# thangktran/HardwareAwareOptimalQuantumCircuitCuttingAndKnitting

Hardware: AMD Instinct MI355X
Metric: subcircuit-instances/s (full-knit wall time = ms_per_step), syc 32 p=2 (higher is better)
Workload: dtype f64

## Files before the change

hardwareawareoptimalquantumcircuitcuttingandknitting_amd/csrc/qknit_prep.hip:

```cpp
#include <hip/hip_runtime.h>

#include <cstdint>
#include <string>

#include "internal.h"

namespace {

typedef double d4_t __attribute__((ext_vector_type(4)));
typedef double d2_t __attribute__((ext_vector_type(2)));

constexpr int PK = 64;
constexpr int PCT = 128;
constexpr int PNP = 16;
constexpr int PTH = 512;
constexpr int XLD = PCT + 2;
constexpr int PG_BLK = 10;
constexpr int PPG = PG_BLK * 256;
constexpr int PPA = PPG;
constexpr int PPB = PPG + PK * PNP;
__host__ __device__ constexpr int prep_tri(int bi, int bj) { return bi * 4 - bi * (bi - 1) / 2 + (bj - bi); }

struct PrepSide {
    const double* Wt;
    const double* q;
    int64_t ldq;
    int64_t N;
    int R;
    double* X;
    const double* P;
};

struct PrepArgs {
    PrepSide s[2];
    int K;
    int split;
    double* part;
};

#ifndef QK_PREP_RS
#define QK_PREP_RS 16
#endif
constexpr int PRS = QK_PREP_RS;
constexpr int PRPW = PRS / 8;
static_assert(PRS % 8 == 0 && PRS >= 8, "stage rows: a multiple of 8 (8 waves)");
#ifndef QK_PREP_NS
#define QK_PREP_NS 2
#endif
#ifndef QK_PREP_WG_PER_CU
#define QK_PREP_WG_PER_CU 2
#endif
#ifndef QK_COMPRESS_COLS
#define QK_COMPRESS_COLS 1
#endif
#ifndef QK_PREP_EXP
#define QK_PREP_EXP 0
#endif
constexpr int PNS = QK_PREP_NS;
#ifndef QK_PREP_QPAD
#define QK_PREP_QPAD 16
#endif
#ifndef QK_PREP_WPAD
#define QK_PREP_WPAD 16
#endif
constexpr int QLD = PCT + QK_PREP_QPAD;
constexpr int WLD = PK + QK_PREP_WPAD;
struct PrepStage {
    double q[PRS][QLD];
    double w[PRS][WLD];
};
union PrepLds {
    PrepStage st[PNS];
    double x[PK][XLD];
};

__device__ __forceinline__ void prep_glds(const double* src, double* lds_row) {
    __builtin_amdgcn_global_load_lds(reinterpret_cast<const void*>(src),
                                     reinterpret_cast<__attribute__((address_space(3))) void*>(
                                         reinterpret_cast<uintptr_t>(lds_row)),
                                     16, 0, 0);
}

__device__ __forceinline__ void prep_vmwait(int n) {
    switch (n < 15 ? n : 15) {
#define QK_PW(k) case k: asm volatile("s_waitcnt vmcnt(" #k ")" ::: "memory"); break;
        QK_PW(0) QK_PW(1) QK_PW(2) QK_PW(3) QK_PW(4) QK_PW(5) QK_PW(6) QK_PW(7)
        QK_PW(8) QK_PW(9) QK_PW(10) QK_PW(11) QK_PW(12) QK_PW(13) QK_PW(14) QK_PW(15)
#undef QK_PW
    }
}

__global__ __launch_bounds__(PTH, 2 * QK_PREP_WG_PER_CU) void qk_prep_operands_kernel(PrepArgs a) {
    __shared__ __attribute__((aligned(16))) PrepLds L;
    const int tid = threadIdx.x, lane = tid & 63, wave = tid >> 6;
    const int l16 = lane & 15, l4 = lane >> 4;
    const int K = a.K;
    int gi0, gj0, gi1 = -1, gj1 = -1;
    switch (wave) {
        case 4: gi0 = 0, gj0 = 1, gi1 = 0, gj1 = 2; break;
        case 5: gi0 = 0, gj0 = 3, gi1 = 1, gj1 = 2; break;
        case 6: gi0 = 1, gj0 = 3; break;
        case 7: gi0 = 2, gj0 = 3; break;
        default: gi0 = gj0 = wave; break;
    }
    gi0 = __builtin_amdgcn_readfirstlane(gi0), gj0 = __builtin_amdgcn_readfirstlane(gj0);
    gi1 = __builtin_amdgcn_readfirstlane(gi1), gj1 = __builtin_amdgcn_readfirstlane(gj1);
    const int wave_s = __builtin_amdgcn_readfirstlane(wave);
    for (int sd = 0; sd < 2; ++sd) {
        const PrepSide& S = a.s[sd];
        const int R = S.R;
        const int nst = (R + PRS - 1) / PRS;
        const int64_t tiles = S.N / PCT;
        d4_t g0 = {0, 0, 0, 0}, g1 = {0, 0, 0, 0}, u = {0, 0, 0, 0};
        const bool mine = !a.split || (int)(blockIdx.x & 1) == sd;
        const int64_t t_first = a.split ? (int64_t)(blockIdx.x >> 1) : (int64_t)blockIdx.x;
        const int64_t t_step = a.split ? (int64_t)(gridDim.x >> 1) : (int64_t)gridDim.x;
        for (int64_t t = mine ? t_first : tiles; t < tiles; t += t_step) {
            const int64_t c0 = t * PCT;
            int nload[PNS];
            auto issue = [&](int st) {
                PrepStage& P = L.st[st % PNS];
                int n = 0;
#pragma unroll
                for (int h = 0; h < PRPW; ++h) {
                    const int rl = PRPW * wave_s + h, r = st * PRS + rl;
                    if (r < R) {
                        prep_glds(S.q + (int64_t)r * S.ldq + c0 + 2 * lane, &P.q[rl][0]);
                        ++n;
                        if (2 * lane < K) prep_glds(S.Wt + (int64_t)r * K + 2 * lane, &P.w[rl][0]);
                        ++n;
                    }
                }
                nload[st % PNS] = n;
            };
            asm volatile("s_waitcnt lgkmcnt(0)" ::: "memory");
            __builtin_amdgcn_s_barrier();
            for (int st = 0; st < PNS - 1 && st < nst; ++st) issue(st);
            d4_t x[4];
#pragma unroll
            for (int i = 0; i < 4; ++i) x[i] = (d4_t){0, 0, 0, 0};
            for (int st = 0; st < ((QK_PREP_EXP & 4) ? 0 : nst); ++st) {
                int after = 0;
                for (int d = st + 1; d < st + PNS - 1 && d < nst; ++d) after += nload[d % PNS];
                prep_vmwait(after);
                asm volatile("s_waitcnt lgkmcnt(0)" ::: "memory");
                __builtin_amdgcn_s_barrier();
                const PrepStage& P = L.st[st % PNS];
                double qb[PRS / 4], wa[PRS / 4][4];
#pragma unroll
                for (int kk = 0; kk < PRS / 4; ++kk) {
                    const int rl = 4 * kk + l4;
                    const bool rv = st * PRS + rl < R;
                    qb[kk] = rv ? P.q[rl][16 * wave + l16] : 0.0;
#pragma unroll
                    for (int i = 0; i < 4; ++i) {
                        const int k = 16 * i + l16;
                        wa[kk][i] = (rv && k < K) ? P.w[rl][k] : 0.0;
                    }
                }
                if (st + PNS - 1 < nst) issue(st + PNS - 1);
#pragma unroll
                for (int kk = 0; kk < PRS / 4; ++kk)
#pragma unroll
                    for (int i = 0; i < 4; ++i) x[i] = __builtin_amdgcn_mfma_f64_16x16x4f64(wa[kk][i], qb[kk], x[i], 0, 0, 0);
            }
            const bool probes = S.P != nullptr && wave < 4;
            constexpr int PPB = 8;
            const double* pp = probes ? S.P + (int64_t)l16 * S.N + c0 + l4 : nullptr;
            double pxn[PPB];
#pragma unroll
            for (int j = 0; j < PPB; ++j) pxn[j] = probes ? pp[4 * j] : 0.0;
            asm volatile("s_waitcnt lgkmcnt(0)" ::: "memory");
            __builtin_amdgcn_s_barrier();
#pragma unroll
            for (int i = 0; i < 4; ++i)
#pragma unroll
                for (int rr = 0; rr < 4; ++rr) L.x[16 * i + l4 + 4 * rr][16 * wave + l16] = x[i][rr];
            asm volatile("s_waitcnt lgkmcnt(0)" ::: "memory");
            __builtin_amdgcn_s_barrier();
            for (int s8 = 0; s8 < ((QK_PREP_EXP & 1) ? 0 : PCT / 4); s8 += PPB) {
                double px[PPB];
#pragma unroll
                for (int j = 0; j < PPB; ++j) px[j] = pxn[j];
                if (probes && s8 + PPB < PCT / 4) {
#pragma unroll
                    for (int j = 0; j < PPB; ++j) pxn[j] = pp[4 * (s8 + PPB + j)];
                }
                if (wave < 4) {
#pragma unroll
                    for (int j = 0; j < PPB; ++j) {
                        const double av = L.x[16 * gi0 + l16][4 * (s8 + j) + l4];
                        g0 = __builtin_amdgcn_mfma_f64_16x16x4f64(av, av, g0, 0, 0, 0);
                        if (probes) u = __builtin_amdgcn_mfma_f64_16x16x4f64(av, px[j], u, 0, 0, 0);
                    }
                } else {
#pragma unroll
                    for (int j = 0; j < PPB; ++j) {
                        const int c = 4 * (s8 + j) + l4;
                        const double a0 = L.x[16 * gi0 + l16][c];
                        const double b0 = L.x[16 * gj0 + l16][c];
                        g0 = __builtin_amdgcn_mfma_f64_16x16x4f64(a0, b0, g0, 0, 0, 0);
                        if (gi1 >= 0) {
                            const double a1 = gi1 == gi0 ? a0 : L.x[16 * gi1 + l16][c];
                            const double b1 = L.x[16 * gj1 + l16][c];
                            g1 = __builtin_amdgcn_mfma_f64_16x16x4f64(a1, b1, g1, 0, 0, 0);
                        }
                    }
                }
            }
            if (!(QK_PREP_EXP & 2)) {
                d2_t z[8];
#pragma unroll
                for (int v = 0; v < 8; ++v) z[v] = *reinterpret_cast<const d2_t*>(&L.x[8 * wave_s + v][2 * lane]);
#pragma unroll
                for (int v = 0; v < 8; ++v)
                    if (8 * wave_s + v < K) *reinterpret_cast<d2_t*>(S.X + (int64_t)(8 * wave_s + v) * S.N + c0 + 2 * lane) = z[v];
            }
        }
        double* p = sd == 0 ? a.part + (int64_t)blockIdx.x * PPA
                            : a.part + (int64_t)gridDim.x * PPA + (int64_t)blockIdx.x * PPB;
#pragma unroll
        for (int rr = 0; rr < 4; ++rr) {
            const int e = (l4 + 4 * rr) * 16 + l16;
            p[prep_tri(gi0, gj0) * 256 + e] = g0[rr];
            if (gi1 >= 0) p[prep_tri(gi1, gj1) * 256 + e] = g1[rr];
            if (sd == 1 && wave < 4) p[PPG + (16 * wave + l4 + 4 * rr) * PNP + l16] = u[rr];
        }
    }
}

constexpr int PRW = 16;
__global__ __launch_bounds__(64 * PRW) void qk_prep_reduce_kernel(const double* __restrict__ part, int nblk,
                                                                  int K, double* __restrict__ GA,
                                                                  double* __restrict__ GB, double* __restrict__ U) {
    __shared__ double acc[PRW][64];
    const int lane = threadIdx.x & 63, grp = threadIdx.x >> 6;
    const int e = blockIdx.x * 64 + lane;
    int sd = -1, off = 0;
    double* dst = nullptr;
    double* mirror = nullptr;
    if (e < 2 * PPG) {
        sd = e < PPG ? 0 : 1;
        off = e - sd * PPG;
        const int blk = off >> 8;
        const int bi = blk < 4 ? 0 : blk < 7 ? 1 : blk < 9 ? 2 : 3;
        const int bj = bi + blk - prep_tri(bi, bi);
        const int r = 16 * bi + ((off >> 4) & 15), c = 16 * bj + (off & 15);
        if (r < K && c < K) {
            double* G = sd == 0 ? GA : GB;
            dst = G + r * K + c;
            if (bi != bj) mirror = G + c * K + r;
        }
    } else if (e < 2 * PPG + PNP * K) {
        const int f = e - 2 * PPG;
        sd = 1, off = PPG + f, dst = U + f;
    }
    if (!dst) sd = -1;
    double s = 0.0;
    if (sd >= 0) {
        const int PPART = sd == 0 ? PPA : PPB;
        const double* p = part + (sd == 0 ? 0 : (int64_t)nblk * PPA) + off;
        double t[8] = {0, 0, 0, 0, 0, 0, 0, 0};
        int b = grp;
        for (; b + 31 * PRW < nblk; b += 32 * PRW) {
            double v[32];
#pragma unroll
            for (int u = 0; u < 32; ++u) v[u] = p[(int64_t)(b + PRW * u) * PPART];
#pragma unroll
            for (int u = 0; u < 32; ++u) t[u & 7] += v[u];
        }
        for (; b < nblk; b += PRW) t[0] += p[(int64_t)b * PPART];
        s = ((t[0] + t[1]) + (t[2] + t[3])) + ((t[4] + t[5]) + (t[6] + t[7]));
    }
    acc[grp][lane] = s;
    __syncthreads();
    if (grp == 0 && dst) {
        double v[PRW];
#pragma unroll
        for (int w = 0; w < PRW; ++w) v[w] = acc[w][lane];
#pragma unroll
        for (int h = PRW / 2; h >= 1; h >>= 1)
#pragma unroll
            for (int w = 0; w < h; ++w) v[w] += v[w + h];
        *dst = v[0];
        if (mirror) *mirror = v[0];
    }
}

__global__ __launch_bounds__(256) void qk_compress_kernel(int K, int rmax, const double* __restrict__ TA,
                                                          const double* __restrict__ XA, int64_t NA, int64_t ldxa,
                                                          double* __restrict__ A2, int64_t lda2,
                                                          const double* __restrict__ TB,
                                                          const double* __restrict__ XB, int64_t NB, int64_t ldxb,
                                                          double* __restrict__ B2, int64_t ldb2) {
    __shared__ double T[8][PK];
    __shared__ double part[4][8][64];
    const bool bs = blockIdx.y == 1;
    const double* Tg = bs ? TB : TA;
    const double* X = bs ? XB : XA;
    double* out = bs ? B2 : A2;
    const int64_t N = bs ? NB : NA, ld = bs ? ldxb : ldxa, ldo = bs ? ldb2 : lda2;
    const int l = threadIdx.x & 63;
    const int q = __builtin_amdgcn_readfirstlane(threadIdx.x >> 6);
    auto load = [&](int64_t c0, double (&xv)[16]) {
        const int64_t c = c0 + l;
#pragma unroll
        for (int u = 0; u < 16; ++u) {
            const int k = 16 * q + u;
            const double* row = X + (int64_t)k * ld;
            xv[u] = (k < K && c < N) ? row[c] : 0.0;
        }
    };
    double xv[16];
    int64_t c0 = (int64_t)blockIdx.x * 64;
    if (c0 < N) load(c0, xv);
    {
        const int n = rmax * K, e0 = threadIdx.x, e1 = threadIdx.x + 256;
        const double t0 = e0 < n ? Tg[e0] : 0.0, t1 = e1 < n ? Tg[e1] : 0.0;
        if (e0 < n) T[e0 / K][e0 % K] = t0;
        if (e1 < n) T[e1 / K][e1 % K] = t1;
    }
    __syncthreads();
    for (; c0 < N; c0 += (int64_t)gridDim.x * 64) {
        double acc[8] = {0, 0, 0, 0, 0, 0, 0, 0};
#pragma unroll
        for (int u = 0; u < 16; ++u)
#pragma unroll
            for (int j = 0; j < 8; ++j)
                if (j < rmax && 16 * q + u < K) acc[j] = fma(T[j][16 * q + u], xv[u], acc[j]);
#pragma unroll
        for (int j = 0; j < 8; ++j) part[q][j][l] = acc[j];
        __syncthreads();
        for (int e = threadIdx.x; e < 8 * 64; e += 256) {
            const int j = e >> 6, cc = e & 63;
            if (j < rmax && c0 + cc < N)
                out[(int64_t)j * ldo + c0 + cc] = (part[0][j][cc] + part[1][j][cc]) + (part[2][j][cc] + part[3][j][cc]);
        }
        __syncthreads();
        if (c0 + (int64_t)gridDim.x * 64 < N) load(c0 + (int64_t)gridDim.x * 64, xv);
    }
}

constexpr int PCW = 16;
__global__ __launch_bounds__(64) void qk_compress_cols_kernel(int K, int rmax, const double* __restrict__ TA,
                                                              const double* __restrict__ XA, int64_t NA, int64_t ldxa,
                                                              double* __restrict__ A2, int64_t lda2,
                                                              const double* __restrict__ TB,
                                                              const double* __restrict__ XB, int64_t NB, int64_t ldxb,
                                                              double* __restrict__ B2, int64_t ldb2) {
    const bool bs = blockIdx.y == 1;
    const double* Tg = bs ? TB : TA;
    const double* X = bs ? XB : XA;
    double* out = bs ? B2 : A2;
    const int64_t N = bs ? NB : NA, ld = bs ? ldxb : ldxa, ldo = bs ? ldb2 : lda2;
    const int64_t c = ((int64_t)blockIdx.x * 64 + threadIdx.x) * 2;
    if ((int64_t)blockIdx.x * 128 >= N) return;
    const int64_t cl = c < N ? c : N - 2;
    d2_t acc[8];
#pragma unroll
    for (int j = 0; j < 8; ++j) acc[j] = (d2_t){0.0, 0.0};
    __shared__ __attribute__((aligned(16))) double Tt[PK][8];
    d2_t buf[2][PCW];
    auto load = [&](int ch, d2_t (&b)[PCW]) {
#pragma unroll
        for (int u = 0; u < PCW; ++u) {
            const int k = min(ch * PCW + u, K - 1);
            b[u] = *reinterpret_cast<const d2_t*>(X + (int64_t)k * ld + cl);
        }
    };
    const int nch = (K + PCW - 1) / PCW;
    {
        double tv[PK * 8 / 64];
#pragma unroll
        for (int i = 0; i < PK * 8 / 64; ++i) {
            const int e = threadIdx.x + 64 * i, k = e >> 3, j = e & 7;
            tv[i] = Tg[min(j, rmax - 1) * K + min(k, K - 1)];
        }
        load(0, buf[0]);
#pragma unroll
        for (int i = 0; i < PK * 8 / 64; ++i) {
            const int e = threadIdx.x + 64 * i, k = e >> 3, j = e & 7;
            Tt[k][j] = (k < K && j < rmax) ? tv[i] : 0.0;
        }
    }
    __syncthreads();
    if (c >= N) return;
#pragma unroll
    for (int ch = 0; ch < PK / PCW; ++ch) {
        if (ch >= nch) break;
        if (ch + 1 < nch) load(ch + 1, buf[(ch + 1) & 1]);
#pragma unroll
        for (int u = 0; u < PCW; ++u) {
            const int k = ch * PCW + u;
            double t[8];
#pragma unroll
            for (int h = 0; h < 4; ++h) {
                const d2_t tv = *reinterpret_cast<const d2_t*>(&Tt[k][2 * h]);
                t[2 * h] = tv.x;
                t[2 * h + 1] = tv.y;
            }
#pragma unroll
            for (int j = 0; j < 8; ++j) {
                acc[j].x = fma(t[j], buf[ch & 1][u].x, acc[j].x);
                acc[j].y = fma(t[j], buf[ch & 1][u].y, acc[j].y);
            }
        }
    }
#pragma unroll
    for (int j = 0; j < 8; ++j)
        if (j < rmax) *reinterpret_cast<d2_t*>(out + (int64_t)j * ldo + c) = acc[j];
}

constexpr int PV_GRID = 128;
constexpr int PV_PART = 8 * 16;

constexpr int CV_COLS = 512;
__global__ __launch_bounds__(256) void qk_compress_v_kernel(int K, int rmax, const double* __restrict__ TA,
                                                            const double* __restrict__ XA, int64_t NA, int64_t ldxa,
                                                            double* __restrict__ A2, int64_t lda2,
                                                            const double* __restrict__ TB,
                                                            const double* __restrict__ XB, int64_t NB, int64_t ldxb,
                                                            double* __restrict__ B2, int64_t ldb2,
                                                            const double* __restrict__ P, int64_t ldp,
                                                            double* __restrict__ vpart, int nA_wg) {
    const int tid = threadIdx.x, lane = tid & 63, wave = tid >> 6;
    const bool bs = (int)blockIdx.x >= nA_wg;
    const int64_t wg = bs ? (int64_t)blockIdx.x - nA_wg : (int64_t)blockIdx.x;
    const double* Tg = bs ? TB : TA;
    const double* X = bs ? XB : XA;
    double* out = bs ? B2 : A2;
    const int64_t N = bs ? NB : NA, ld = bs ? ldxb : ldxa, ldo = bs ? ldb2 : lda2;
    const int64_t base = wg * CV_COLS + wave * 128;
    const int64_t c = base + 2 * lane;
    const bool valid = c < N;
    const int64_t cl = valid ? c : N - 2;
    __shared__ __attribute__((aligned(16))) double Tt[PK][8];
    __shared__ __attribute__((aligned(16))) double Bt[4][8][128 + 2];
    __shared__ double Vw[4][PV_PART];
    d2_t acc[8];
#pragma unroll
    for (int j = 0; j < 8; ++j) acc[j] = (d2_t){0.0, 0.0};
    d2_t buf[2][PCW];
    auto load = [&](int ch, d2_t (&b)[PCW]) {
#pragma unroll
        for (int u = 0; u < PCW; ++u) {
            const int k = min(ch * PCW + u, K - 1);
            b[u] = *reinterpret_cast<const d2_t*>(X + (int64_t)k * ld + cl);
        }
    };
    const int nch = (K + PCW - 1) / PCW;
    {
        double tv[2];
#pragma unroll
        for (int i = 0; i < 2; ++i) {
            const int e = tid + 256 * i, k = e >> 3, j = e & 7;
            tv[i] = Tg[min(j, rmax - 1) * K + min(k, K - 1)];
        }
        if (base < N) load(0, buf[0]);
#pragma unroll
        for (int i = 0; i < 2; ++i) {
            const int e = tid + 256 * i, k = e >> 3, j = e & 7;
            Tt[k][j] = (k < K && j < rmax) ? tv[i] : 0.0;
        }
    }
    __syncthreads();
    if (base < N) {
#pragma unroll
        for (int ch = 0; ch < PK / PCW; ++ch) {
            if (ch >= nch) break;
            if (ch + 1 < nch) load(ch + 1, buf[(ch + 1) & 1]);
#pragma unroll
            for (int u = 0; u < PCW; ++u) {
                const int k = ch * PCW + u;
                double t[8];
#pragma unroll
                for (int h = 0; h < 4; ++h) {
                    const d2_t tv = *reinterpret_cast<const d2_t*>(&Tt[k][2 * h]);
                    t[2 * h] = tv.x;
                    t[2 * h + 1] = tv.y;
                }
#pragma unroll
                for (int j = 0; j < 8; ++j) {
                    acc[j].x = fma(t[j], buf[ch & 1][u].x, acc[j].x);
                    acc[j].y = fma(t[j], buf[ch & 1][u].y, acc[j].y);
                }
            }
        }
        if (valid) {
#pragma unroll
            for (int j = 0; j < 8; ++j)
                if (j < rmax) *reinterpret_cast<d2_t*>(out + (int64_t)j * ldo + c) = acc[j];
        }
    }
    if (!bs) return;
#pragma unroll
    for (int j = 0; j < 8; ++j) {
        const d2_t v = (valid && j < rmax) ? acc[j] : (d2_t){0.0, 0.0};
        *reinterpret_cast<d2_t*>(&Bt[wave][j][2 * lane]) = v;
    }
    __syncthreads();
    const int i16 = lane & 15, k4 = lane >> 4;
    d4_t va = {0.0, 0.0, 0.0, 0.0};
    if (base < N) {
        constexpr int VB = 8;
        const double* pr = P + (int64_t)i16 * ldp;
#pragma unroll
        for (int s0 = 0; s0 < 32; s0 += VB) {
            double pb[VB];
#pragma unroll
            for (int s = 0; s < VB; ++s) {
                const int64_t col = base + 4 * (s0 + s) + k4;
                pb[s] = col < N ? pr[col] : 0.0;
            }
#pragma unroll
            for (int s = 0; s < VB; ++s) {
                const double a = i16 < 8 ? Bt[wave][i16][4 * (s0 + s) + k4] : 0.0;
                va = __builtin_amdgcn_mfma_f64_16x16x4f64(a, pb[s], va, 0, 0, 0);
            }
        }
    }
#pragma unroll
    for (int r = 0; r < 2; ++r) Vw[wave][(k4 + 4 * r) * 16 + i16] = va[r];
    __syncthreads();
    if (tid < PV_PART)
        vpart[wg * PV_PART + tid] = (Vw[0][tid] + Vw[1][tid]) + (Vw[2][tid] + Vw[3][tid]);
}

__global__ __launch_bounds__(256) void qk_probe_v_kernel(int rmax, const double* __restrict__ B2, int64_t ldb2,
                                                         int64_t NB, const double* __restrict__ P, int64_t ldp,
                                                         double* __restrict__ vpart) {
    const int tid = threadIdx.x, lane = tid & 63, wave = tid >> 6;
    double acc[8][4];
#pragma unroll
    for (int jj = 0; jj < 8; ++jj)
#pragma unroll
        for (int q = 0; q < 4; ++q) acc[jj][q] = 0.0;
    struct Col {
        double b[8], pv[4];
    };
    const int64_t step = (int64_t)gridDim.x * 64;
    auto fetch = [&](int64_t c, Col& x) {
        const int64_t cc = c < NB ? c : NB - 1;
#pragma unroll
        for (int jj = 0; jj < 8; ++jj) x.b[jj] = B2[(int64_t)min(jj, rmax - 1) * ldb2 + cc];
#pragma unroll
        for (int q = 0; q < 4; ++q) x.pv[q] = P[(int64_t)(4 * wave + q) * ldp + cc];
    };
    auto mac = [&](const Col& x) {
#pragma unroll
        for (int jj = 0; jj < 8; ++jj)
#pragma unroll
            for (int q = 0; q < 4; ++q) acc[jj][q] = fma(x.b[jj], x.pv[q], acc[jj][q]);
    };
    int64_t c = (int64_t)blockIdx.x * 64 + lane;
    if (c < NB) {
        Col x0, x1;
        fetch(c, x0);
        for (;; c += 2 * step) {
            fetch(c + step, x1);
            __builtin_amdgcn_sched_barrier(0);
            mac(x0);
            if (c + step >= NB) break;
            fetch(c + 2 * step, x0);
            __builtin_amdgcn_sched_barrier(0);
            mac(x1);
            if (c + 2 * step >= NB) break;
        }
    }
#pragma unroll
    for (int jj = 0; jj < 8; ++jj)
#pragma unroll
        for (int q = 0; q < 4; ++q) {
            double v = acc[jj][q];
#pragma unroll
            for (int s = 1; s < 64; s <<= 1) v += __shfl_xor(v, s, 64);
            acc[jj][q] = jj < rmax ? v : 0.0;
        }
    double* out = vpart + (int64_t)blockIdx.x * PV_PART;
    if (lane < 32) {
        const int j8 = lane >> 2, q = lane & 3;
        double v = 0.0;
#pragma unroll
        for (int jj = 0; jj < 8; ++jj)
#pragma unroll
            for (int qq = 0; qq < 4; ++qq)
                if (jj == j8 && qq == q) v = acc[jj][qq];
        out[j8 * 16 + 4 * wave + q] = v;
    }
}

__global__ __launch_bounds__(256) void qk_probe_d_kernel(int K, int rmax, const double* __restrict__ XA, int64_t ldx,
                                                         int64_t NA, const double* __restrict__ A2, int64_t lda2,
                                                         const double* __restrict__ U,
                                                         const double* __restrict__ vpart, int gv,
                                                         double* __restrict__ epart) {
    __shared__ double Us[PK][PNP];
    __shared__ double Vs[16][PNP];
    __shared__ double ep[4][2 * PNP];
    const int tid = threadIdx.x, lane = tid & 63, wave = tid >> 6, l16 = lane & 15, l4 = lane >> 4;
    {
        __shared__ double vh[PV_PART];
        const int e = tid & (PV_PART - 1), h = tid >> 7;
        double t[16];
#pragma unroll
        for (int u = 0; u < 16; ++u) t[u] = 0.0;
        int b = h;
        for (; b + 30 < gv; b += 32) {
            double v[16];
#pragma unroll
            for (int u = 0; u < 16; ++u) v[u] = vpart[(int64_t)(b + 2 * u) * PV_PART + e];
#pragma unroll
            for (int u = 0; u < 16; ++u) t[u] += v[u];
        }
        for (; b < gv; b += 2) t[0] += vpart[(int64_t)b * PV_PART + e];
#pragma unroll
        for (int w = 8; w >= 1; w >>= 1)
#pragma unroll
            for (int u = 0; u < w; ++u) t[u] += t[u + w];
        if (h == 1) vh[e] = t[0];
        __syncthreads();
        if (h == 0) Vs[e / 16][e % 16] = -(t[0] + vh[e]);
        else Vs[8 + e / 16][e % 16] = 0.0;
    }
    for (int e = tid; e < PK * PNP; e += 256) Us[e / PNP][e % PNP] = (e / PNP) < K ? U[e] : 0.0;
    __syncthreads();
    double e2 = 0.0, f2 = 0.0;
    for (int64_t cb = (int64_t)blockIdx.x * 4 + wave; cb * 16 < NA; cb += (int64_t)gridDim.x * 4) {
        const int64_t c = cb * 16 + l16;
        double av[PK / 4], a2[2];
#pragma unroll
        for (int kk = 0; kk < PK / 4; ++kk) av[kk] = XA[(int64_t)min(4 * kk + l4, K - 1) * ldx + c];
#pragma unroll
        for (int jj = 0; jj < 2; ++jj) a2[jj] = A2[(int64_t)min(4 * jj + l4, rmax - 1) * lda2 + c];
        d4_t acc = {0, 0, 0, 0};
#pragma unroll
        for (int kk = 0; kk < PK / 4; ++kk)
            acc = __builtin_amdgcn_mfma_f64_16x16x4f64(av[kk], Us[4 * kk + l4][l16], acc, 0, 0, 0);
#pragma unroll
        for (int rr = 0; rr < 4; ++rr) f2 = fma(acc[rr], acc[rr], f2);
#pragma unroll
        for (int jj = 0; jj < 2; ++jj)
            acc = __builtin_amdgcn_mfma_f64_16x16x4f64(a2[jj], Vs[4 * jj + l4][l16], acc, 0, 0, 0);
#pragma unroll
        for (int rr = 0; rr < 4; ++rr) e2 = fma(acc[rr], acc[rr], e2);
    }
    e2 += __shfl_xor(e2, 16, 64);
    e2 += __shfl_xor(e2, 32, 64);
    f2 += __shfl_xor(f2, 16, 64);
    f2 += __shfl_xor(f2, 32, 64);
    if (l4 == 0) {
        ep[wave][l16] = e2;
        ep[wave][PNP + l16] = f2;
    }
    __syncthreads();
    if (tid < 2 * PNP)
        epart[(int64_t)blockIdx.x * 2 * PNP + tid] = ep[0][tid] + ep[1][tid] + ep[2][tid] + ep[3][tid];
}

constexpr int PE = 2 * PNP;

__global__ __launch_bounds__(256) void qk_probe_accept_kernel(const double* __restrict__ epart, int n,
                                                              const int32_t* __restrict__ r_dev, double tol,
                                                              double rel_tol, double* __restrict__ e2_out,
                                                              int32_t* __restrict__ k_out, double* __restrict__ err_out,
                                                              int64_t* __restrict__ tally = nullptr) {
    __shared__ double acc[256];
    const int tid = threadIdx.x, p = tid % PE;
    constexpr int STEP = 256 / PE;
    double s8[8] = {0, 0, 0, 0, 0, 0, 0, 0};
    int b = tid / PE;
    for (; b + 31 * STEP < n; b += 32 * STEP) {
        double v[32];
#pragma unroll
        for (int u = 0; u < 32; ++u) v[u] = epart[(int64_t)(b + u * STEP) * PE + p];
#pragma unroll
        for (int u = 0; u < 32; ++u) s8[u & 7] += v[u];
    }
    for (; b < n; b += STEP) s8[0] += epart[(int64_t)b * PE + p];
    const double s = ((s8[0] + s8[1]) + (s8[2] + s8[3])) + ((s8[4] + s8[5]) + (s8[6] + s8[7]));
    acc[tid] = s;
    __syncthreads();
    for (int w = 128; w >= PE; w >>= 1) {
        if (tid < w) acc[tid] += acc[tid + w];
        __syncthreads();
    }
    if (tid < PE && e2_out) e2_out[tid] = acc[tid];
    if (tid == 0 && k_out) {
        double m = 0.0, f = 0.0;
        for (int q = 0; q < PNP; ++q) {
            m = fmax(m, acc[q]);
            f = fmax(f, acc[PNP + q]);
        }
        const double err = sqrt(m);
        const double bound = fmax(tol, rel_tol * sqrt(f));
        const int r = *r_dev;
        if (err_out) *err_out = err;
        const int k = (r > 0 && err <= bound) ? r : 0;
        *k_out = k;
        if (tally) {
            tally[0] += r == 0 ? 1 : 0;
            tally[1] += (r > 0 && k == 0) ? 1 : 0;
            tally[2] = k;
            tally[3] += 1;
        }
    }
}

int probe_grid_d(qk_ctx* ctx, int64_t NA) {
    const int64_t blocks = (NA + 63) / 64;
    const int64_t cap = (int64_t)(ctx->cus > 0 ? ctx->cus : 256) * 2;
    return (int)(blocks < cap ? (blocks > 0 ? blocks : 1) : cap);
}

int fail(qk_ctx* ctx, int code, const char* msg) {
    ctx->err = msg;
    return code;
}

#ifndef QK_PREP_SPLIT
#define QK_PREP_SPLIT 1
#endif
bool prep_split(qk_ctx* ctx, int64_t NA, int64_t NB) {
    const int64_t tiles = (NA > NB ? NA : NB) / PCT;
    const int64_t g = (int64_t)(ctx->cus > 0 ? ctx->cus : 256) * QK_PREP_WG_PER_CU;
    return QK_PREP_SPLIT && tiles > 0 && 2 * tiles <= g;
}

int prep_grid(qk_ctx* ctx, int64_t NA, int64_t NB) {
    const int64_t tiles = (NA > NB ? NA : NB) / PCT;
    if (prep_split(ctx, NA, NB)) return (int)(2 * tiles);
    const int64_t g = (int64_t)(ctx->cus > 0 ? ctx->cus : 256) * QK_PREP_WG_PER_CU;
    return (int)(tiles < g ? (tiles > 0 ? tiles : 1) : g);
}

}

extern "C" {

int qk_prep_workspace_bytes(qk_ctx* ctx, int64_t NA, int64_t NB, int64_t* bytes) {
    if (!ctx || !bytes) return QK_EARG;
    *bytes = (int64_t)prep_grid(ctx, NA, NB) * (PPA + PPB) * (int64_t)sizeof(double);
    return QK_OK;
}

int qk_prep_operands(qk_ctx* ctx, int K, int RA, const double* WtA, const double* qA, int64_t ldqA, int64_t NA,
                     double* XA, int RB, const double* WtB, const double* qB, int64_t ldqB, int64_t NB, double* XB,
                     const double* probes, double* GA, double* GB, double* U, double* work, int64_t work_bytes) {
    if (!ctx) return QK_EARG;
    if (K < 2 || K > PK || (K & 1) || RA < 1 || RB < 1)
        return fail(ctx, QK_EARG, "qk_prep_operands: need even 2 <= K <= 64 and R >= 1 on both sides");
    if (((reinterpret_cast<uintptr_t>(WtA) | reinterpret_cast<uintptr_t>(WtB) | reinterpret_cast<uintptr_t>(qA) |
          reinterpret_cast<uintptr_t>(qB)) & 15) || (ldqA & 1) || (ldqB & 1))
        return fail(ctx, QK_EARG, "qk_prep_operands: 16-B aligned Wt / q and even ldq required");
    if (NA < PCT || NB < PCT || NA % PCT || NB % PCT || ldqA < NA || ldqB < NB)
        return fail(ctx, QK_EARG, "qk_prep_operands: columns must be a positive multiple of 128 (ldq >= N)");
    if (!WtA || !qA || !XA || !WtB || !qB || !XB || !probes || !GA || !GB || !U || !work)
        return fail(ctx, QK_EARG, "qk_prep_operands: null buffer");
    const int G = prep_grid(ctx, NA, NB);
    if (work_bytes < (int64_t)G * (PPA + PPB) * (int64_t)sizeof(double))
        return fail(ctx, QK_EARG, "qk_prep_operands: workspace too small (qk_prep_workspace_bytes)");
    if (hipSetDevice(ctx->device) != hipSuccess) return fail(ctx, QK_EHIP, "qk_prep_operands: hipSetDevice");
    PrepArgs args;
    args.s[0] = PrepSide{WtA, qA, ldqA, NA, RA, XA, nullptr};
    args.s[1] = PrepSide{WtB, qB, ldqB, NB, RB, XB, probes};
    args.K = K;
    args.split = prep_split(ctx, NA, NB) ? 1 : 0;
    args.part = work;
    hipLaunchKernelGGL(qk_prep_operands_kernel, dim3(G), dim3(PTH), 0, ctx->stream, args);
    const int outs = 2 * PPG + PNP * K;
    hipLaunchKernelGGL(qk_prep_reduce_kernel, dim3((outs + 63) / 64), dim3(64 * PRW), 0, ctx->stream, work, G, K, GA,
                       GB, U);
    const hipError_t e = hipGetLastError();
    if (e != hipSuccess) return fail(ctx, QK_EHIP, (std::string("qk_prep_operands: ") + hipGetErrorString(e)).c_str());
    return QK_OK;
}

int qk_compress_operands(qk_ctx* ctx, int K, int rmax, const double* TA, const double* XA, int64_t NA, double* A2,
                         const double* TB, const double* XB, int64_t NB, double* B2) {
    return qk_compress_operands_ld(ctx, K, rmax, TA, XA, NA, NA, A2, NA, TB, XB, NB, NB, B2, NB);
}

int qk_compress_operands_ld(qk_ctx* ctx, int K, int rmax, const double* TA, const double* XA, int64_t NA, int64_t ldxa,
                            double* A2, int64_t lda2, const double* TB, const double* XB, int64_t NB, int64_t ldxb,
                            double* B2, int64_t ldb2) {
    if (!ctx) return QK_EARG;
    if (K < 1 || K > PK || rmax < 1 || rmax > 8 || NA < 1 || NB < 1)
        return fail(ctx, QK_EARG, "qk_compress_operands: need 1 <= K <= 64, 1 <= rmax <= 8, N >= 1");
    if (ldxa < NA || lda2 < NA || ldxb < NB || ldb2 < NB)
        return fail(ctx, QK_EARG, "qk_compress_operands: leading dimension below the width");
    if (!TA || !XA || !A2 || !TB || !XB || !B2) return fail(ctx, QK_EARG, "qk_compress_operands: null buffer");
    if (hipSetDevice(ctx->device) != hipSuccess) return fail(ctx, QK_EHIP, "qk_compress_operands: hipSetDevice");
    const int64_t N = NA > NB ? NA : NB;
    const bool cols = QK_COMPRESS_COLS && NA % 2 == 0 && NB % 2 == 0 && ldxa % 2 == 0 && lda2 % 2 == 0 &&
                      ldxb % 2 == 0 && ldb2 % 2 == 0 &&
                      !((reinterpret_cast<uintptr_t>(XA) | reinterpret_cast<uintptr_t>(XB) |
                         reinterpret_cast<uintptr_t>(A2) | reinterpret_cast<uintptr_t>(B2)) & 15);
    if (cols) {
        hipLaunchKernelGGL(qk_compress_cols_kernel, dim3((unsigned)((N + 127) / 128), 2), dim3(64), 0, ctx->stream, K,
                           rmax, TA, XA, NA, ldxa, A2, lda2, TB, XB, NB, ldxb, B2, ldb2);
    } else {
        int64_t gx = (N + 63) / 64;
        const int64_t cap = (int64_t)(ctx->cus > 0 ? ctx->cus : 256) * 4;
        gx = gx < cap ? gx : cap;
        hipLaunchKernelGGL(qk_compress_kernel, dim3((unsigned)gx, 2), dim3(256), 0, ctx->stream, K, rmax, TA, XA, NA,
                           ldxa, A2, lda2, TB, XB, NB, ldxb, B2, ldb2);
    }
    const hipError_t e = hipGetLastError();
    if (e != hipSuccess)
        return fail(ctx, QK_EHIP, (std::string("qk_compress_operands: ") + hipGetErrorString(e)).c_str());
    return QK_OK;
}

int qk_compress_probe_v(qk_ctx* ctx, int K, int rmax, const double* TA, const double* XA, int64_t NA, int64_t ldxa,
                        double* A2, int64_t lda2, const double* TB, const double* XB, int64_t NB, int64_t ldxb,
                        double* B2, int64_t ldb2, const double* probes, int64_t ldp, double* vpart,
                        int64_t vpart_doubles) {
    if (!ctx) return QK_EARG;
    if (K < 1 || K > PK || rmax < 1 || rmax > 8 || NA < 2 || NB < 2 || (NA | NB | ldxa | lda2 | ldxb | ldb2) & 1)
        return fail(ctx, QK_EARG, "qk_compress_probe_v: need 1 <= K <= 64, 1 <= rmax <= 8, even widths and strides");
    if (ldxa < NA || lda2 < NA || ldxb < NB || ldb2 < NB || ldp < NB)
        return fail(ctx, QK_EARG, "qk_compress_probe_v: leading dimension below the width");
    if (!TA || !XA || !A2 || !TB || !XB || !B2 || !probes || !vpart)
        return fail(ctx, QK_EARG, "qk_compress_probe_v: null buffer");
    if ((reinterpret_cast<uintptr_t>(XA) | reinterpret_cast<uintptr_t>(XB) | reinterpret_cast<uintptr_t>(A2) |
         reinterpret_cast<uintptr_t>(B2)) & 15)
        return fail(ctx, QK_EARG, "qk_compress_probe_v: operands must be 16-B aligned");
    const int64_t ga = (NA + CV_COLS - 1) / CV_COLS, gb = (NB + CV_COLS - 1) / CV_COLS;
    if (vpart_doubles < gb * PV_PART) return fail(ctx, QK_EARG, "qk_compress_probe_v: vpart too small");
    if (hipSetDevice(ctx->device) != hipSuccess) return fail(ctx, QK_EHIP, "qk_compress_probe_v: hipSetDevice");
    hipLaunchKernelGGL(qk_compress_v_kernel, dim3((unsigned)(ga + gb)), dim3(256), 0, ctx->stream, K, rmax, TA, XA, NA,
                       ldxa, A2, lda2, TB, XB, NB, ldxb, B2, ldb2, probes, ldp, vpart, (int)ga);
    const hipError_t e = hipGetLastError();
    if (e != hipSuccess)
        return fail(ctx, QK_EHIP, (std::string("qk_compress_probe_v: ") + hipGetErrorString(e)).c_str());
    return QK_OK;
}

int qk_probe_errors_vpart(qk_ctx* ctx, int K, int rmax, const double* XA, int64_t ldx, int64_t NA, const double* A2,
                          int64_t lda2, const double* U, const double* vpart, int64_t gv, double* e2,
                          const int32_t* r_dev, double tol, double rel_tol, int32_t* k_out, double* err_out,
                          double* work, int64_t work_bytes, int64_t* tally) {
    if (!ctx) return QK_EARG;
    if (K < 1 || K > PK || rmax < 1 || rmax > 8 || NA < 16 || NA % 16 || gv < 1)
        return fail(ctx, QK_EARG, "qk_probe_errors_vpart: need 1 <= K <= 64, 1 <= rmax <= 8, NA % 16 == 0, gv >= 1");
    if (!XA || !A2 || !U || !vpart || !work || (k_out && !r_dev) || (tally && !k_out))
        return fail(ctx, QK_EARG, "qk_probe_errors_vpart: null buffer");
    if (ldx < NA) return fail(ctx, QK_EARG, "qk_probe_errors_vpart: leading dimension");
    const int gd = probe_grid_d(ctx, NA);
    if (work_bytes < (int64_t)(PV_GRID * PV_PART + gd * PE) * (int64_t)sizeof(double))
        return fail(ctx, QK_EARG, "qk_probe_errors_vpart: workspace too small (qk_probe_workspace_bytes)");
    if (hipSetDevice(ctx->device) != hipSuccess) return fail(ctx, QK_EHIP, "qk_probe_errors_vpart: hipSetDevice");
    double* epart = work + PV_GRID * PV_PART;
    hipLaunchKernelGGL(qk_probe_d_kernel, dim3(gd), dim3(256), 0, ctx->stream, K, rmax, XA, ldx, NA, A2, lda2, U, vpart,
                       (int)gv, epart);
    hipLaunchKernelGGL(qk_probe_accept_kernel, dim3(1), dim3(256), 0, ctx->stream, epart, gd, r_dev, tol, rel_tol, e2,
                       k_out, err_out, tally);
    const hipError_t e = hipGetLastError();
    if (e != hipSuccess)
        return fail(ctx, QK_EHIP, (std::string("qk_probe_errors_vpart: ") + hipGetErrorString(e)).c_str());
    return QK_OK;
}

int qk_probe_workspace_bytes(qk_ctx* ctx, int64_t NA, int64_t* bytes) {
    if (!ctx || !bytes) return QK_EARG;
    *bytes = (int64_t)(PV_GRID * PV_PART + probe_grid_d(ctx, NA) * PE) * (int64_t)sizeof(double);
    return QK_OK;
}

int qk_probe_errors(qk_ctx* ctx, int K, int rmax, const double* XA, int64_t ldx, int64_t NA, const double* A2,
                    int64_t lda2, const double* U, const double* B2, int64_t ldb2, int64_t NB, const double* probes,
                    int64_t ldp, double* e2, const int32_t* r_dev, double tol, double rel_tol, int32_t* k_out,
                    double* err_out, double* work, int64_t work_bytes) {
    return qk_probe_errors_tally(ctx, K, rmax, XA, ldx, NA, A2, lda2, U, B2, ldb2, NB, probes, ldp, e2, r_dev, tol,
                                 rel_tol, k_out, err_out, work, work_bytes, nullptr);
}

int qk_probe_errors_tally(qk_ctx* ctx, int K, int rmax, const double* XA, int64_t ldx, int64_t NA, const double* A2,
                          int64_t lda2, const double* U, const double* B2, int64_t ldb2, int64_t NB,
                          const double* probes, int64_t ldp, double* e2, const int32_t* r_dev, double tol,
                          double rel_tol, int32_t* k_out, double* err_out, double* work, int64_t work_bytes,
                          int64_t* tally) {
    if (!ctx) return QK_EARG;
    if (K < 1 || K > PK || rmax < 1 || rmax > 8 || NA < 16 || NA % 16 || NB < 4 || NB % 4)
        return fail(ctx, QK_EARG, "qk_probe_errors: need 1 <= K <= 64, 1 <= rmax <= 8, NA % 16 == 0, NB % 4 == 0");
    if (!XA || !A2 || !U || !B2 || !probes || !work || (k_out && !r_dev) || (tally && !k_out))
        return fail(ctx, QK_EARG, "qk_probe_errors: null buffer");
    if (ldx < NA || ldb2 < NB || ldp < NB) return fail(ctx, QK_EARG, "qk_probe_errors: leading dimension");
    const int gd = probe_grid_d(ctx, NA);
    if (work_bytes < (int64_t)(PV_GRID * PV_PART + gd * PE) * (int64_t)sizeof(double))
        return fail(ctx, QK_EARG, "qk_probe_errors: workspace too small (qk_probe_workspace_bytes)");
    if (hipSetDevice(ctx->device) != hipSuccess) return fail(ctx, QK_EHIP, "qk_probe_errors: hipSetDevice");
    double* vpart = work;
    double* epart = work + PV_GRID * PV_PART;
    hipLaunchKernelGGL(qk_probe_v_kernel, dim3(PV_GRID), dim3(256), 0, ctx->stream, rmax, B2, ldb2, NB, probes, ldp,
                       vpart);
    hipLaunchKernelGGL(qk_probe_d_kernel, dim3(gd), dim3(256), 0, ctx->stream, K, rmax, XA, ldx, NA, A2, lda2, U, vpart,
                       PV_GRID, epart);
    hipLaunchKernelGGL(qk_probe_accept_kernel, dim3(1), dim3(256), 0, ctx->stream, epart, gd, r_dev, tol, rel_tol, e2,
                       k_out, err_out, tally);
    const hipError_t e = hipGetLastError();
    if (e != hipSuccess) return fail(ctx, QK_EHIP, (std::string("qk_probe_errors: ") + hipGetErrorString(e)).c_str());
    return QK_OK;
}

__global__ __launch_bounds__(64) void qk_rank_tally_kernel(const int32_t* __restrict__ r, const int32_t* __restrict__ k,
                                                          int64_t* __restrict__ acc) {
    if (threadIdx.x == 0) {
        const int rv = *r, kv = *k;
        acc[0] += rv == 0 ? 1 : 0;
        acc[1] += (rv > 0 && kv == 0) ? 1 : 0;
        acc[2] = kv;
        acc[3] += 1;
    }
}

int qk_rank_tally(qk_ctx* ctx, const int32_t* r_dev, const int32_t* k_dev, int64_t* acc) {
    if (!ctx) return QK_EARG;
    if (!r_dev || !k_dev || !acc) return fail(ctx, QK_EARG, "qk_rank_tally: null buffer");
    if (hipSetDevice(ctx->device) != hipSuccess) return fail(ctx, QK_EHIP, "qk_rank_tally: hipSetDevice");
    hipLaunchKernelGGL(qk_rank_tally_kernel, dim3(1), dim3(64), 0, ctx->stream, r_dev, k_dev, acc);
    const hipError_t e = hipGetLastError();
    if (e != hipSuccess) return fail(ctx, QK_EHIP, (std::string("qk_rank_tally: ") + hipGetErrorString(e)).c_str());
    return QK_OK;
}

int qk_probe_accept(qk_ctx* ctx, const double* e2, int n, const int32_t* r_dev, double tol, double rel_tol,
                    int32_t* k_out, double* err_out) {
    if (!ctx) return QK_EARG;
    if (!e2 || !r_dev || !k_out || n < 1) return fail(ctx, QK_EARG, "qk_probe_accept: null buffer or n < 1");
    if (hipSetDevice(ctx->device) != hipSuccess) return fail(ctx, QK_EHIP, "qk_probe_accept: hipSetDevice");
    hipLaunchKernelGGL(qk_probe_accept_kernel, dim3(1), dim3(256), 0, ctx->stream, e2, n, r_dev, tol, rel_tol, nullptr,
                       k_out, err_out);
    const hipError_t e = hipGetLastError();
    if (e != hipSuccess) return fail(ctx, QK_EHIP, (std::string("qk_probe_accept: ") + hipGetErrorString(e)).c_str());
    return QK_OK;
}

}
```

Baseline: 517,800.

## Skip zero rows of compression matrix via ballot pivot mask in compress kernels

The compress kernels now build a ballot mask of the K rows of the small transform T that have any nonzero entry. They load and accumulate only those rows of X, with a double-buffered chunk loop of width 8. The prep MFMA loop also breaks early on row groups beyond R. This cuts global loads and FMAs when T is sparse, at the cost of data-dependent indexing, serial bit scans and less regular prefetching.

```diff
diff --git a/hardwareawareoptimalquantumcircuitcuttingandknitting_amd/csrc/qknit_prep.hip b/hardwareawareoptimalquantumcircuitcuttingandknitting_amd/csrc/qknit_prep.hip
--- a/hardwareawareoptimalquantumcircuitcuttingandknitting_amd/csrc/qknit_prep.hip
+++ b/hardwareawareoptimalquantumcircuitcuttingandknitting_amd/csrc/qknit_prep.hip
@@ -160,9 +160,11 @@
                 }
                 if (st + PNS - 1 < nst) issue(st + PNS - 1);
 #pragma unroll
-                for (int kk = 0; kk < PRS / 4; ++kk)
+                for (int kk = 0; kk < PRS / 4; ++kk) {
+                    if (st * PRS + 4 * kk >= R) break;
 #pragma unroll
                     for (int i = 0; i < 4; ++i) x[i] = __builtin_amdgcn_mfma_f64_16x16x4f64(wa[kk][i], qb[kk], x[i], 0, 0, 0);
+                }
             }
             const bool probes = S.P != nullptr && wave < 4;
             constexpr int PPB = 8;
@@ -287,6 +289,8 @@
     }
 }
 
+constexpr int PCW = 8;
+
 __global__ __launch_bounds__(256) void qk_compress_kernel(int K, int rmax, const double* __restrict__ TA,
                                                           const double* __restrict__ XA, int64_t NA, int64_t ldxa,
                                                           double* __restrict__ A2, int64_t lda2,
@@ -302,18 +306,6 @@
     const int64_t N = bs ? NB : NA, ld = bs ? ldxb : ldxa, ldo = bs ? ldb2 : lda2;
     const int l = threadIdx.x & 63;
     const int q = __builtin_amdgcn_readfirstlane(threadIdx.x >> 6);
-    auto load = [&](int64_t c0, double (&xv)[16]) {
-        const int64_t c = c0 + l;
-#pragma unroll
-        for (int u = 0; u < 16; ++u) {
-            const int k = 16 * q + u;
-            const double* row = X + (int64_t)k * ld;
-            xv[u] = (k < K && c < N) ? row[c] : 0.0;
-        }
-    };
-    double xv[16];
-    int64_t c0 = (int64_t)blockIdx.x * 64;
-    if (c0 < N) load(c0, xv);
     {
         const int n = rmax * K, e0 = threadIdx.x, e1 = threadIdx.x + 256;
         const double t0 = e0 < n ? Tg[e0] : 0.0, t1 = e1 < n ? Tg[e1] : 0.0;
@@ -321,13 +313,36 @@
         if (e1 < n) T[e1 / K][e1 % K] = t1;
     }
     __syncthreads();
+    bool nz = false;
+    if (l < K)
+        for (int j = 0; j < rmax; ++j) nz |= T[j][l] != 0.0;
+    uint64_t m = __ballot(nz);
+    for (int s = 0; s < 16 * q && m; ++s) m &= m - 1;
+    int ks[16], cnt = 0;
+#pragma unroll
+    for (int u = 0; u < 16; ++u) {
+        ks[u] = m ? (int)__builtin_ctzll(m | (1ull << 63)) : 0;
+        cnt += m != 0;
+        m &= m - 1;
+    }
+    auto load = [&](int64_t c0, double (&xv)[16]) {
+        const int64_t c = c0 + l;
+#pragma unroll
+        for (int u = 0; u < 16; ++u) {
+            const double* row = X + (int64_t)ks[u] * ld;
+            xv[u] = (u < cnt && c < N) ? row[c] : 0.0;
+        }
+    };
+    double xv[16];
+    int64_t c0 = (int64_t)blockIdx.x * 64;
+    if (c0 < N) load(c0, xv);
     for (; c0 < N; c0 += (int64_t)gridDim.x * 64) {
         double acc[8] = {0, 0, 0, 0, 0, 0, 0, 0};
 #pragma unroll
         for (int u = 0; u < 16; ++u)
 #pragma unroll
             for (int j = 0; j < 8; ++j)
-                if (j < rmax && 16 * q + u < K) acc[j] = fma(T[j][16 * q + u], xv[u], acc[j]);
+                if (j < rmax && u < cnt) acc[j] = fma(T[j][ks[u]], xv[u], acc[j]);
 #pragma unroll
         for (int j = 0; j < 8; ++j) part[q][j][l] = acc[j];
         __syncthreads();
@@ -341,7 +356,68 @@
     }
 }
 
-constexpr int PCW = 16;
+__device__ __forceinline__ uint64_t compress_pivots(const double (*Tt)[8], int lane) {
+    bool nz = false;
+#pragma unroll
+    for (int h = 0; h < 4; ++h) {
+        const d2_t tv = *reinterpret_cast<const d2_t*>(&Tt[lane][2 * h]);
+        nz |= tv.x != 0.0 || tv.y != 0.0;
+    }
+    return __ballot(nz);
+}
+
+__device__ __forceinline__ void compress_rows(const double (*Tt)[8], uint64_t m, const double* __restrict__ X,
+                                              int64_t ld, int64_t cl, d2_t (&acc)[8]) {
+    d2_t b0[PCW], b1[PCW];
+    int k0[PCW], k1[PCW];
+    auto load = [&](d2_t (&b)[PCW], int (&ks)[PCW]) {
+        int n = 0, k = 0;
+#pragma unroll
+        for (int u = 0; u < PCW; ++u) {
+            k = m ? (int)__builtin_ctzll(m | (1ull << 63)) : k;
+            n += m != 0;
+            m &= m - 1;
+            ks[u] = k;
+            b[u] = *reinterpret_cast<const d2_t*>(X + (int64_t)k * ld + cl);
+        }
+        return n;
+    };
+    auto sum = [&](const d2_t (&b)[PCW], const int (&ks)[PCW], int n) {
+#pragma unroll
+        for (int u = 0; u < PCW; ++u) {
+            if (u >= n) break;
+            double t[8];
+#pragma unroll
+            for (int h = 0; h < 4; ++h) {
+                const d2_t tv = *reinterpret_cast<const d2_t*>(&Tt[ks[u]][2 * h]);
+                t[2 * h] = tv.x;
+                t[2 * h + 1] = tv.y;
+            }
+#pragma unroll
+            for (int j = 0; j < 8; ++j) {
+                acc[j].x = fma(t[j], b[u].x, acc[j].x);
+                acc[j].y = fma(t[j], b[u].y, acc[j].y);
+            }
+        }
+    };
+    if (!m) return;
+    int n0 = load(b0, k0), n1;
+    for (;;) {
+        if (!m) {
+            sum(b0, k0, n0);
+            break;
+        }
+        n1 = load(b1, k1);
+        sum(b0, k0, n0);
+        if (!m) {
+            sum(b1, k1, n1);
+            break;
+        }
+        n0 = load(b0, k0);
+        sum(b1, k1, n1);
+    }
+}
+
 __global__ __launch_bounds__(64) void qk_compress_cols_kernel(int K, int rmax, const double* __restrict__ TA,
                                                               const double* __restrict__ XA, int64_t NA, int64_t ldxa,
                                                               double* __restrict__ A2, int64_t lda2,
@@ -360,15 +436,6 @@
 #pragma unroll
     for (int j = 0; j < 8; ++j) acc[j] = (d2_t){0.0, 0.0};
     __shared__ __attribute__((aligned(16))) double Tt[PK][8];
-    d2_t buf[2][PCW];
-    auto load = [&](int ch, d2_t (&b)[PCW]) {
-#pragma unroll
-        for (int u = 0; u < PCW; ++u) {
-            const int k = min(ch * PCW + u, K - 1);
-            b[u] = *reinterpret_cast<const d2_t*>(X + (int64_t)k * ld + cl);
-        }
-    };
-    const int nch = (K + PCW - 1) / PCW;
     {
         double tv[PK * 8 / 64];
 #pragma unroll
@@ -376,7 +443,6 @@
             const int e = threadIdx.x + 64 * i, k = e >> 3, j = e & 7;
             tv[i] = Tg[min(j, rmax - 1) * K + min(k, K - 1)];
         }
-        load(0, buf[0]);
 #pragma unroll
         for (int i = 0; i < PK * 8 / 64; ++i) {
             const int e = threadIdx.x + 64 * i, k = e >> 3, j = e & 7;
@@ -384,28 +450,8 @@
         }
     }
     __syncthreads();
+    compress_rows(Tt, compress_pivots(Tt, threadIdx.x), X, ld, cl, acc);
     if (c >= N) return;
-#pragma unroll
-    for (int ch = 0; ch < PK / PCW; ++ch) {
-        if (ch >= nch) break;
-        if (ch + 1 < nch) load(ch + 1, buf[(ch + 1) & 1]);
-#pragma unroll
-        for (int u = 0; u < PCW; ++u) {
-            const int k = ch * PCW + u;
-            double t[8];
-#pragma unroll
-            for (int h = 0; h < 4; ++h) {
-                const d2_t tv = *reinterpret_cast<const d2_t*>(&Tt[k][2 * h]);
-                t[2 * h] = tv.x;
-                t[2 * h + 1] = tv.y;
-            }
-#pragma unroll
-            for (int j = 0; j < 8; ++j) {
-                acc[j].x = fma(t[j], buf[ch & 1][u].x, acc[j].x);
-                acc[j].y = fma(t[j], buf[ch & 1][u].y, acc[j].y);
-            }
-        }
-    }
 #pragma unroll
     for (int j = 0; j < 8; ++j)
         if (j < rmax) *reinterpret_cast<d2_t*>(out + (int64_t)j * ldo + c) = acc[j];
@@ -440,15 +486,6 @@
     d2_t acc[8];
 #pragma unroll
     for (int j = 0; j < 8; ++j) acc[j] = (d2_t){0.0, 0.0};
-    d2_t buf[2][PCW];
-    auto load = [&](int ch, d2_t (&b)[PCW]) {
-#pragma unroll
-        for (int u = 0; u < PCW; ++u) {
-            const int k = min(ch * PCW + u, K - 1);
-            b[u] = *reinterpret_cast<const d2_t*>(X + (int64_t)k * ld + cl);
-        }
-    };
-    const int nch = (K + PCW - 1) / PCW;
     {
         double tv[2];
 #pragma unroll
@@ -456,7 +493,6 @@
             const int e = tid + 256 * i, k = e >> 3, j = e & 7;
             tv[i] = Tg[min(j, rmax - 1) * K + min(k, K - 1)];
         }
-        if (base < N) load(0, buf[0]);
 #pragma unroll
         for (int i = 0; i < 2; ++i) {
             const int e = tid + 256 * i, k = e >> 3, j = e & 7;
@@ -464,28 +500,9 @@
         }
     }
     __syncthreads();
+    const uint64_t piv = compress_pivots(Tt, lane);
     if (base < N) {
-#pragma unroll
-        for (int ch = 0; ch < PK / PCW; ++ch) {
-            if (ch >= nch) break;
-            if (ch + 1 < nch) load(ch + 1, buf[(ch + 1) & 1]);
-#pragma unroll
-            for (int u = 0; u < PCW; ++u) {
-                const int k = ch * PCW + u;
-                double t[8];
-#pragma unroll
-                for (int h = 0; h < 4; ++h) {
-                    const d2_t tv = *reinterpret_cast<const d2_t*>(&Tt[k][2 * h]);
-                    t[2 * h] = tv.x;
-                    t[2 * h + 1] = tv.y;
-                }
-#pragma unroll
-                for (int j = 0; j < 8; ++j) {
-                    acc[j].x = fma(t[j], buf[ch & 1][u].x, acc[j].x);
-                    acc[j].y = fma(t[j], buf[ch & 1][u].y, acc[j].y);
-                }
-            }
-        }
+        compress_rows(Tt, piv, X, ld, cl, acc);
         if (valid) {
 #pragma unroll
             for (int j = 0; j < 8; ++j)
```

New measurement: 519,100, median of 6. No clear change (+0.2%).
